# bwa-mem2/bwa-mem2

Hardware: NVIDIA H100
Metric: paired 151bp reads/s (seed+chain+extend hot path) (higher is better)
Workload: dtype int64/int16

## Files before the change

bwa-mem2_b200/csrc/pipeline.cu:

```cuda
#include "bm2_common.cuh"
#include "bm2_ctx.h"
#include "fm_device.cuh"
#include "chain_device.cuh"
#include "ext_device.cuh"
#include <cub/device/device_radix_sort.cuh>
#include <cub/device/device_scan.cuh>
#include <vector>
#include <algorithm>
#include <mutex>
#include <thread>
#include <string>
#include <cstring>
#include <cstdlib>
#include <cmath>

static_assert(sizeof(ExtJobRec) == sizeof(BswJob), "ExtJobRec must alias BswJob");

int bsw_launch_with_scratch(bm2_ctx *ctx_for_error, cudaStream_t stream, const BswJob *d_jobs, BswOut *d_out, int n,
                            const uint8_t *d_tbase, const uint8_t *d_qbase, const BswParams &prm,
                            unsigned long long *d_cells, void *scratch, size_t scratch_bytes, int wide_possible);

__global__ void occ_relayout_kernel(ulonglong2 *tab, size_t n_entries) {
    const size_t i = (size_t) blockIdx.x * blockDim.x + threadIdx.x;
    if (i >= n_entries) return;
// ... 369 lines not shown
    const int r = perm[t];
    const int64_t c0 = chain_off[r], c1 = chain_off[r + 1];
    if (c1 == c0) return;
    const int64_t g0 = reg_off[r];
    ext_build_read_d(cv, ep, chains + c0, (int) (c1 - c0), seeds, (int) (offs[r + 1] - offs[r]), offs[r], c0, g0, b.regs + g0,
                     b.reg_chain + g0, b.reg_seed + g0, b.left + left_off[r], b.left_reg + left_off[r], b.right + right_off[r],
                     b.right_reg + right_off[r], b.srt + g0, b.state ? b.state + g0 : nullptr);
}

__global__ void right_h0_kernel(ExtJobRec *jobs, const int32_t *job_reg, int n, const bm2_alnreg_t *regs) {
    int i = blockIdx.x * blockDim.x + threadIdx.x;
    if (i < n) jobs[i].h0 = regs[job_reg[i]].score;
}

__global__ void fold_kernel(ExtParams ep, const ExtJobRec *jobs, const int32_t *job_reg, const BswOut *outs, const int32_t *sel, int n,
                            int is_right, int w, int last_try, bm2_alnreg_t *regs, const int32_t *reg_chain, const bm2_chain *chains,
                            const bm2_seed *seeds, const int64_t *offs, int32_t *retry, Counters *cnt)
{
    int t = blockIdx.x * blockDim.x + threadIdx.x;
    if (t >= n) return;
    const int j = sel ? sel[t] : t;
    const BswOut o = outs[t];
    const int g = job_reg[j];
    const bm2_chain c = chains[reg_chain[g]];
    const int l_query = (int) (offs[c.seqid + 1] - offs[c.seqid]);
    bm2_alnreg_t a = regs[g];
    const bool ok = ext_fold_d(ep, a, is_right, jobs[j].h0, o.score, o.qle, o.tle, o.gtle, o.gscore, o.max_off, w, last_try, l_query,
                               seeds + c.seed_off, c.n_seeds);
    regs[g] = a;
    if (!ok) { unsigned long long k = atomicAdd(&cnt->n_retry, 1ULL); retry[k] = j; }
}

__global__ void gather_jobs_kernel(const ExtJobRec *jobs, const int32_t *sel, int n, ExtJobRec *out) {
    int t = blockIdx.x * blockDim.x + threadIdx.x;
    if (t < n) out[t] = jobs[sel[t]];
}

__global__ void ext_select_kernel(const ExtJobRec *__restrict__ jobs, const int32_t *__restrict__ job_reg, int n,
                                  const uint8_t *__restrict__ state, int last, ExtJobRec *out, int32_t *out_reg, unsigned long long *n_out)
{
    const int i = blockIdx.x * blockDim.x + threadIdx.x, lane = threadIdx.x & 31;
    int g = 0;
    bool take = false;
    if (i < n) { g = job_reg[i]; const uint8_t s = state[g]; take = s == EXT_NEED || (last && s == EXT_TODO); }
    const unsigned m = __ballot_sync(0xffffffffu, take);
    if (!m) return;
    const int leader = __ffs(m) - 1;
    unsigned long long at = 0;
    if (lane == leader) at = atomicAdd(n_out, (unsigned long long) __popc(m));
    at = __shfl_sync(0xffffffffu, at, leader);
    if (take) { const unsigned long long k = at + __popc(m & ((1u << lane) - 1u)); out[k] = jobs[i]; out_reg[k] = g; }
}

__global__ void ext_mark_done_kernel(uint8_t *state, int64_t n) {
    const int64_t i = (int64_t) blockIdx.x * blockDim.x + threadIdx.x;
    if (i < n && state[i] == EXT_NEED) state[i] = EXT_DONE;
}

__global__ void __launch_bounds__(128)
ext_walk_kernel(ExtParams ep, const bm2_chain *__restrict__ chains, const bm2_seed *__restrict__ seeds, const int64_t *__restrict__ chain_off,
                const int64_t *__restrict__ reg_off, const int64_t *__restrict__ offs, int n_reads, const bm2_alnreg_t *regs,
                const int32_t *__restrict__ reg_seed, uint8_t *state, int32_t *srt2_all, PfBox *box_all, PfCursor *cur, int first, int heavy,
                Counters *cnt)
{
    const int r = blockIdx.x * blockDim.x + threadIdx.x;
    bool done = false;
    if (r < n_reads) {
        const int64_t c0 = chain_off[r], c1 = chain_off[r + 1], g0 = reg_off[r];
        const int n_reg = (int) (reg_off[r + 1] - g0), n_chain = (int) (c1 - c0);
        if (n_chain > 0 && n_reg <= heavy) {
            PfCursor c;
            if (first) { c.ci = 0; c.k = -1; c.lim = 0; c.base = 0; } else c = cur[r];
            if (c.ci < n_chain) {
                done = ext_walk_read_d(ep, chains + c0, n_chain, seeds, (int) (offs[r + 1] - offs[r]), regs + g0, n_reg, reg_seed + g0,
                                       state + g0, srt2_all + g0, box_all + g0, c);
                cur[r] = c;
            }
        }
    }
    if (first) {
        const unsigned m = __ballot_sync(0xffffffffu, done);
        if ((threadIdx.x & 31) == 0 && m) atomicAdd(&cnt->n_walk_done, (unsigned long long) __popc(m));
    }
}

__device__ void ext_postfilter_read_warp(const ExtParams &p, const bm2_chain *chains, int n_chain, const bm2_seed *seeds, int l_query,
                                         bm2_alnreg_t *regs, int n_reg, const int32_t *reg_seed, int32_t *srt2, PfBox *box)
{
    const int lane = threadIdx.x & 31;
    for (int i = lane; i < n_reg; i += 32) box[i] = pf_box_d(regs[i]);
    __syncwarp();
    int lim = 0, base = 0;
    for (int ci = 0; ci < n_chain; ++ci) {
        const bm2_chain &c = chains[ci];
        const bm2_seed *cs = seeds + c.seed_off;
        const int n = c.n_seeds;
        if (n == 0) continue;
        for (int k = n - 1 - lane; k >= 0; k -= 32) srt2[k] = reg_seed[base + (n - 1 - k)];
        __syncwarp();
        for (int k = n - 1; k >= 0; --k) {
            const bm2_seed s = cs[srt2[k]];
            int v = 0;
            bool hit = false;
            for (int i0 = 0; i0 < n_reg && v < lim && !hit; i0 += 128) {
                int kind[4];
#pragma unroll
                for (int g = 0; g < 4; ++g) {
                    const int i = i0 + 32 * g + lane;
                    kind[g] = i < n_reg ? pf_box_kind_d(p, s, box[i], l_query) : 0;
                }
#pragma unroll
                for (int g = 0; g < 4; ++g) {
                    const unsigned cm = __ballot_sync(0xFFFFFFFFu, kind[g] == 1), hm = __ballot_sync(0xFFFFFFFFu, kind[g] == 2);
                    if (hit || v >= lim || i0 + 32 * g >= n_reg) continue;
                    if (hm) {
                        const int at = v + __popc(cm & ((1u << (__ffs(hm) - 1)) - 1u));
                        if (at < lim) { v = at; hit = true; continue; }
                    }
                    v += __popc(cm);
                }
            }
            if (v < lim) {
                if (!pf_chain_overlap_d(cs, n, srt2, k, s)) {
                    __syncwarp();
                    if (lane == 0) {
                        const int ai = base + (n - 1 - k);
                        regs[ai].qb = regs[ai].qe = -1;
                        box[ai].qb = box[ai].qe = -1;
                        srt2[k] = -1;
                    }
                    __syncwarp();
                    continue;
                }
            }
            lim++;
        }
        __syncwarp();
        base += n;
    }
}


__device__ int tail_compact_warp(bm2_alnreg_t *a, int n, int lane) {
    int m = 0;
    for (int i0 = 0; i0 < n; i0 += 32) {
        const int i = i0 + lane;
        uint4 v[7];
        bool keep = false;
        if (i < n) {
            const uint4 *s4 = reinterpret_cast<const uint4 *>(a + i);
#pragma unroll
            for (int k = 0; k < 7; ++k) v[k] = s4[k];
            keep = a[i].qe > a[i].qb;
        }
        const unsigned km = __ballot_sync(0xffffffffu, keep);
        __syncwarp();
        if (keep) {
            const int d = m + __popc(km & ((1u << lane) - 1u));
            if (d != i) {
                uint4 *d4 = reinterpret_cast<uint4 *>(a + d);
#pragma unroll
                for (int k = 0; k < 7; ++k) d4[k] = v[k];
            }
        }
        m += __popc(km);
        __syncwarp();
    }
    return m;
}

__device__ void tail_permute_warp(bm2_alnreg_t *a, int32_t *idx, int n, int lane) {
    for (int i = 0; i < n; ++i) {
        const int first = idx[i];
        if (first < 0 || first == i) continue;
        uint4 tmp = make_uint4(0, 0, 0, 0);
        if (lane < 7) tmp = reinterpret_cast<const uint4 *>(a + i)[lane];
        int j = i;
        for (;;) {
            const int src = idx[j];
            __syncwarp();
            if (lane == 0) idx[j] = -1;
            if (src == i) { if (lane < 7) reinterpret_cast<uint4 *>(a + j)[lane] = tmp; break; }
            if (lane < 7) reinterpret_cast<uint4 *>(a + j)[lane] = reinterpret_cast<const uint4 *>(a + src)[lane];
            j = src;
        }
        __syncwarp();
    }
}

__device__ int ext_tail_read_warp(const ContigView &cv, const ExtParams &p, const uint8_t *ref, const uint8_t *query, bm2_alnreg_t *a, int n_reg,
                                  int32_t *he, int32_t *idx, TailSortKey *keys)
{
    const int lane = threadIdx.x & 31;
    int n = tail_compact_warp(a, n_reg, lane);
    if (n > 1) {
        for (int i = lane; i < n; i += 32) { idx[i] = i; keys[i].r = a[i].re; }
        __syncwarp();
        if (lane == 0) {
            const TailSortKey *rk = keys;
            ks_introsort_d(idx, (long) n, [rk](int x, int y) { return rk[x].r < rk[y].r; });
        }
        __syncwarp();
        tail_permute_warp(a, idx, n, lane);
        for (int i = lane; i < n; i += 32) reg_set_n_comp_d(a[i], 1);
        __syncwarp();
        if (lane == 0) sort_dedup_scan_d(cv, p, ref, query, n, a, he);
        __syncwarp();
        n = tail_compact_warp(a, n, lane);
        for (int i = lane; i < n; i += 32) { idx[i] = i; keys[i].r = a[i].rb; keys[i].score = a[i].score; keys[i].qb = a[i].qb; }
        __syncwarp();
        if (lane == 0) {
            const TailSortKey *rk = keys;
            ks_introsort_d(idx, (long) n, [rk](int xi, int yi) {
                const TailSortKey x = rk[xi], y = rk[yi];
                return x.score > y.score || (x.score == y.score && (x.r < y.r || (x.r == y.r && x.qb < y.qb)));
            });
        }
        __syncwarp();
        tail_permute_warp(a, idx, n, lane);
        for (int i0 = 0; i0 < n; i0 += 32) {
            const int i = i0 + lane;
            const bool dup = i >= 1 && i < n && a[i].score == a[i - 1].score && a[i].rb == a[i - 1].rb && a[i].qb == a[i - 1].qb;
            __syncwarp();
            if (dup) a[i].qe = a[i].qb;
        }
        __syncwarp();
        if (n > 1) n = 1 + tail_compact_warp(a + 1, n - 1, lane);
    }
    for (int i = lane; i < n; i += 32)
        if (a[i].rid >= 0 && cv.ann_alt && cv.ann_alt[a[i].rid]) reg_set_is_alt_d(a[i], 1);
    __syncwarp();
    return n;
}

template <int mode>
__global__ void __launch_bounds__(128, mode ? 4 : 1)
tail_kernel(ContigView cv, ExtParams ep, const uint8_t *__restrict__ ref, const uint8_t *__restrict__ codes, const int64_t *__restrict__ offs,
            const bm2_chain *__restrict__ chains, const bm2_seed *__restrict__ seeds, const int64_t *__restrict__ chain_off,
            const int64_t *__restrict__ reg_off, int n_reads, bm2_alnreg_t *regs, const int32_t *reg_seed, int32_t *srt2_all, int32_t *he_all,
            int he_stride, const int32_t *__restrict__ perm, PfBox *box_all, int32_t *n_final, int heavy_thr, int light_sorted, int coop_tail)
{
    const int tid = blockIdx.x * blockDim.x + threadIdx.x, nthr = gridDim.x * blockDim.x;
    const int lane = threadIdx.x & 31;
    int32_t *he = he_all + (size_t) (mode ? tid >> 5 : tid) * he_stride;
    const int unit = mode ? tid >> 5 : tid, nunit = mode ? nthr >> 5 : nthr;
    for (int t = unit; t < n_reads; t += nunit) {
        const int r = (mode || light_sorted) ? perm[t] : t;
        const int64_t c0 = chain_off[r], c1 = chain_off[r + 1], g0 = reg_off[r];
        const int n_reg = (int) (reg_off[r + 1] - g0);
        if (mode) { if (n_reg <= heavy_thr) break; }
        else if (n_reg > heavy_thr) continue;
        int m = 0;
        if (c1 > c0) {
            const int l_query = (int) (offs[r + 1] - offs[r]);
            if (mode) {
                ext_postfilter_read_warp(ep, chains + c0, (int) (c1 - c0), seeds, l_query, regs + g0, n_reg, reg_seed + g0, srt2_all + g0, box_all + g0);
                __syncwarp();
                if (coop_tail) m = ext_tail_read_warp(cv, ep, ref, codes + offs[r], regs + g0, n_reg, he, srt2_all + g0, reinterpret_cast<TailSortKey *>(box_all + g0));
                else if (lane == 0) m = ext_tail_read_d(cv, ep, ref, codes + offs[r], regs + g0, n_reg, he, srt2_all + g0, reinterpret_cast<TailSortKey *>(box_all + g0));
                __syncwarp();
            } else {
                ext_postfilter_read_d(ep, chains + c0, (int) (c1 - c0), seeds, l_query, regs + g0, n_reg, reg_seed + g0, srt2_all + g0, box_all + g0);
                m = ext_tail_read_d(cv, ep, ref, codes + offs[r], regs + g0, n_reg, he, srt2_all + g0, reinterpret_cast<TailSortKey *>(box_all + g0));
            }
        }
        if (!mode || lane == 0) n_final[r] = m;
    }
}

__global__ void regs_gather_kernel(const bm2_alnreg_t *regs, const int64_t *reg_off, const int64_t *out_off, int n_reads, bm2_alnreg_t *out) {
    const int r = blockIdx.x * blockDim.x + threadIdx.x;
    if (r >= n_reads) return;
    const int64_t o0 = out_off[r], o1 = out_off[r + 1], g0 = reg_off[r];
    for (int64_t k = 0; k < o1 - o0; ++k) reg_copy(&out[o0 + k], &regs[g0 + k]);
}

__global__ void work_keys_slots_kernel(const int64_t *read_smem_off, const int64_t *slot_off, int n, uint32_t *keys, int32_t *vals) {
    int r = blockIdx.x * blockDim.x + threadIdx.x;
    if (r >= n) return;
    int64_t w = slot_off[read_smem_off[r + 1]] - slot_off[read_smem_off[r]];
    keys[r] = 0xFFFFFFFFu - (uint32_t) (w > 0x7FFFFFFF ? 0x7FFFFFFF : w);
    vals[r] = r;
}
__global__ void work_keys_off_kernel(const int64_t *off, int n, uint32_t *keys, int32_t *vals) {
    int r = blockIdx.x * blockDim.x + threadIdx.x;
    if (r >= n) return;
    int64_t w = off[r + 1] - off[r];
    keys[r] = 0xFFFFFFFFu - (uint32_t) (w > 0x7FFFFFFF ? 0x7FFFFFFF : w);
    vals[r] = r;
}

__global__ void widen_kernel(const int32_t *in, int n, int64_t *out) {
    int i = blockIdx.x * blockDim.x + threadIdx.x;
    if (i < n) out[i] = in[i];
    if (i == n) out[i] = 0;
}

namespace {
enum Buf {
    B_CODES, B_OFFS, B_CNT, B_PREV, B_RESEED, B_SMEM_RAW, B_KEYS_IN, B_KEYS_OUT, B_VALS_IN, B_VALS_OUT, B_CUB, B_SMEM, B_SLOT_CNT,
    B_SLOT_OFF, B_READ_SMEM_OFF, B_SA, B_WSEED, B_WCHAIN, B_ORD, B_SRT, B_KV, B_FIN_CHAIN, B_FIN_SEED, B_PER_READ, B_SCAN, B_CHAINS,
    B_SEEDS, B_REGS, B_REG_AUX, B_JOBS, B_NW, B_OUT, B_PERM, B_ORDPOS, B_FLT, B_MINHSP, B_OWNER, B_POOL, B_TASKS, B_RTASKS, B_COUNT_
};
static_assert(B_COUNT_ <= 64, "bm2_ctx::d[] too small");
enum HBuf { H_OUT_REGS, H_OUT_OFF, H_SMEM, H_CHAINS, H_SEEDS, H_MISC };

struct Stages {
    bm2_ctx *ctx; std::vector<cudaEvent_t> &ev; std::vector<const char *> &names;
    int n = 0;
    int mark(const char *name) {
        bm2_ctx *ctx_for_error = ctx;
        if ((int) ev.size() <= n) { cudaEvent_t e; BM2_CUDA_OK(cudaEventCreate(&e)); ev.push_back(e); }
        BM2_CUDA_OK(cudaEventRecord(ev[n], ctx->stream));
        if ((int) names.size() <= n) names.push_back(name); else names[n] = name;
        ++n;
// ... 241 lines not shown
    char *prb = (char *) ctx->d[B_PER_READ].p;
    int32_t *d_nchain = (int32_t *) prb, *d_nseed = (int32_t *) (prb + pr), *d_nleft = (int32_t *) (prb + 2 * pr),
            *d_nright = (int32_t *) (prb + 3 * pr), *d_nfinal = (int32_t *) (prb + 4 * pr);
    ChainBufs cb = { P<WSeed>(ctx, B_WSEED), P<WChain>(ctx, B_WCHAIN), P<int32_t>(ctx, B_ORD), P<int32_t>(ctx, B_SRT), P<int32_t>(ctx, B_KV),
                     P<int64_t>(ctx, B_ORDPOS), P<FltRec>(ctx, B_FLT),
                     P<bm2_chain>(ctx, B_FIN_CHAIN), P<bm2_seed>(ctx, B_FIN_SEED), d_nchain, d_nseed, d_nleft, d_nright };
    if (ctx->ensure(ctx->d[B_PERM], al((size_t) n * 4) * 4)) return 1;
    uint32_t *wk_in = (uint32_t *) ctx->d[B_PERM].p, *wk_out = (uint32_t *) ((char *) ctx->d[B_PERM].p + al((size_t) n * 4));
    int32_t *wv_in = (int32_t *) ((char *) ctx->d[B_PERM].p + 2 * al((size_t) n * 4)), *d_perm = (int32_t *) ((char *) ctx->d[B_PERM].p + 3 * al((size_t) n * 4));
    work_keys_slots_kernel<<<(n + 255) / 256, 256, 0, st>>>(P<int64_t>(ctx, B_READ_SMEM_OFF), P<int64_t>(ctx, B_SLOT_OFF), n, wk_in, wv_in);
    if (sort_work(ctx, wk_in, wk_out, wv_in, d_perm, n, true)) return 1;
    const int light_sorted = env_int("BM2_LIGHT_SORTED", 0, 0, 1);
    const int chain_heavy = env_int("BM2_CHAIN_HEAVY", 64, 1, 1 << 30);
    const int chain_coop_min = env_int("BM2_CHAIN_COOP_MIN", 1024, 0, 1 << 30);
    chain_kernel<<<(n + 127) / 128, 128, 0, st>>>(pv.cv, pv.cp, P<bm2_smem>(ctx, B_SMEM), P<int64_t>(ctx, B_READ_SMEM_OFF),
                                                  P<int64_t>(ctx, B_SLOT_OFF), P<int64_t>(ctx, B_SA), d_offs, n, d_perm, cb, pv.sw, ctx->idx.ref, d_codes,
                                                  any_flt ? P<int32_t>(ctx, B_MINHSP) : nullptr, 0, chain_heavy, chain_coop_min, light_sorted);
    {
        int heavy_warps = n < ctx->n_sm * 256 ? n : ctx->n_sm * 256;
        chain_kernel<<<(heavy_warps * 32 + 127) / 128, 128, 0, st>>>(pv.cv, pv.cp, P<bm2_smem>(ctx, B_SMEM), P<int64_t>(ctx, B_READ_SMEM_OFF),
                                                                      P<int64_t>(ctx, B_SLOT_OFF), P<int64_t>(ctx, B_SA), d_offs, n, d_perm, cb, pv.sw,
                                                                      ctx->idx.ref, d_codes, any_flt ? P<int32_t>(ctx, B_MINHSP) : nullptr, 1, chain_heavy, chain_coop_min, 0);
    }

    if (sg.mark("compact")) return 1;
    const size_t sc = al((size_t) (n + 2) * 8);
    char *scb = (char *) ctx->d[B_SCAN].p;
    int64_t *w_tmp = (int64_t *) scb, *d_chain_off = (int64_t *) (scb + sc), *d_reg_off = (int64_t *) (scb + 2 * sc),
            *d_left_off = (int64_t *) (scb + 3 * sc), *d_right_off = (int64_t *) (scb + 4 * sc), *d_out_off = (int64_t *) (scb + 5 * sc);
    const int gw = (n + 1 + 255) / 256;
    widen_kernel<<<gw, 256, 0, st>>>(d_nchain, n, w_tmp); if (scan64(ctx, w_tmp, d_chain_off, n)) return 1;
    widen_kernel<<<gw, 256, 0, st>>>(d_nseed, n, w_tmp);  if (scan64(ctx, w_tmp, d_reg_off, n)) return 1;
    widen_kernel<<<gw, 256, 0, st>>>(d_nleft, n, w_tmp);  if (scan64(ctx, w_tmp, d_left_off, n)) return 1;
    widen_kernel<<<gw, 256, 0, st>>>(d_nright, n, w_tmp); if (scan64(ctx, w_tmp, d_right_off, n)) return 1;
    int64_t tot[4];
    BM2_CUDA_OK(cudaMemcpyAsync(&tot[0], d_chain_off + n, 8, cudaMemcpyDeviceToHost, st));
    BM2_CUDA_OK(cudaMemcpyAsync(&tot[1], d_reg_off + n, 8, cudaMemcpyDeviceToHost, st));
    BM2_CUDA_OK(cudaMemcpyAsync(&tot[2], d_left_off + n, 8, cudaMemcpyDeviceToHost, st));
    BM2_CUDA_OK(cudaMemcpyAsync(&tot[3], d_right_off + n, 8, cudaMemcpyDeviceToHost, st));
    BM2_CUDA_OK(cudaMemcpyAsync(&h_cnt, d_cnt, sizeof(Counters), cudaMemcpyDeviceToHost, st));
    BM2_CUDA_OK(cudaStreamSynchronize(st));
    ctx->last_n_lf = h_cnt.n_lf;
    const int64_t n_chains = tot[0], n_regs = tot[1], n_left = tot[2], n_right = tot[3];
    bs.n_chains = n_chains; bs.n_regs = n_regs; bs.n_left = n_left; bs.n_right = n_right;
    if (n_regs > 2000000000LL) { bm2_set_error(ctx, "too many seeds in one batch"); return 1; }
    if (ctx->ensure(ctx->d[B_CHAINS], (size_t) (n_chains + 1) * sizeof(bm2_chain)) || ctx->ensure(ctx->d[B_SEEDS], (size_t) (n_regs + 1) * sizeof(bm2_seed))) return 1;
    chain_compact_kernel<<<(n + 127) / 128, 128, 0, st>>>(P<int64_t>(ctx, B_READ_SMEM_OFF), P<int64_t>(ctx, B_SLOT_OFF), n, P<bm2_chain>(ctx, B_FIN_CHAIN),
                                                          P<bm2_seed>(ctx, B_FIN_SEED), d_chain_off, d_reg_off, P<bm2_chain>(ctx, B_CHAINS), P<bm2_seed>(ctx, B_SEEDS));
    if (upto == UPTO_CHAIN) { if (sg.mark("end")) return 1; BM2_CUDA_OK(cudaStreamSynchronize(st)); return 0; }

    if (sg.mark("extbuild")) return 1;
    const size_t nr1 = (size_t) n_regs + 1, nl1 = (size_t) n_left + 1, nrt1 = (size_t) n_right + 1;
    const int lazy = env_int("BM2_EXT_LAZY", 1, 0, 1);
    const int waves = env_int("BM2_EXT_WAVES", 2, 2, 64);
    const size_t aux_bytes = al(nr1 * 4) * 3 + al(nr1 * 8) + al(nl1 * 4) * 2 + al(nrt1 * 4) * 2 + al(nr1 * sizeof(PfBox)) +
                             (lazy ? al(nr1) + al((size_t) n * sizeof(PfCursor)) + al(nl1 * 4) + al(nrt1 * 4) : 0);
    const size_t njmax = nl1 > nrt1 ? nl1 : nrt1;
    if (ctx->ensure(ctx->d[B_REGS], nr1 * sizeof(bm2_alnreg_t)) || ctx->ensure(ctx->d[B_REG_AUX], aux_bytes) ||
        ctx->ensure(ctx->d[B_JOBS], al(nl1 * sizeof(ExtJobRec)) + al(nrt1 * sizeof(ExtJobRec)) + al(njmax * sizeof(ExtJobRec)) + al(njmax * sizeof(BswOut)) +
                                    (lazy ? al(nl1 * sizeof(ExtJobRec)) + al(nrt1 * sizeof(ExtJobRec)) : 0)) ||
        ctx->ensure(ctx->bsw_scratch, bsw_scratch_bytes((int) njmax))) return 1;
    char *ab = (char *) ctx->d[B_REG_AUX].p;
    int32_t *d_reg_chain = (int32_t *) ab; ab += al(nr1 * 4);
    int32_t *d_reg_seed = (int32_t *) ab; ab += al(nr1 * 4);
    int32_t *d_srt2 = (int32_t *) ab; ab += al(nr1 * 4);
    uint64_t *d_srt = (uint64_t *) ab; ab += al(nr1 * 8);
    int32_t *d_left_reg = (int32_t *) ab; ab += al(nl1 * 4);
    int32_t *d_left_retry = (int32_t *) ab; ab += al(nl1 * 4);
    int32_t *d_right_reg = (int32_t *) ab; ab += al(nrt1 * 4);
    int32_t *d_right_retry = (int32_t *) ab; ab += al(nrt1 * 4);
    PfBox *d_box = (PfBox *) ab; ab += al(nr1 * sizeof(PfBox));
    uint8_t *d_state = nullptr; PfCursor *d_cursor = nullptr; int32_t *d_wleft_reg = nullptr, *d_wright_reg = nullptr;
    if (lazy) {
        d_state = (uint8_t *) ab; ab += al(nr1);
        d_cursor = (PfCursor *) ab; ab += al((size_t) n * sizeof(PfCursor));
        d_wleft_reg = (int32_t *) ab; ab += al(nl1 * 4);
        d_wright_reg = (int32_t *) ab; ab += al(nrt1 * 4);
    }
    char *jb = (char *) ctx->d[B_JOBS].p;
    ExtJobRec *d_left = (ExtJobRec *) jb; jb += al(nl1 * sizeof(ExtJobRec));
    ExtJobRec *d_right = (ExtJobRec *) jb; jb += al(nrt1 * sizeof(ExtJobRec));
    ExtJobRec *d_retry_jobs = (ExtJobRec *) jb; jb += al(njmax * sizeof(ExtJobRec));
    BswOut *d_outs = (BswOut *) jb; jb += al(njmax * sizeof(BswOut));
    ExtJobRec *d_wleft = nullptr, *d_wright = nullptr;
    if (lazy) { d_wleft = (ExtJobRec *) jb; jb += al(nl1 * sizeof(ExtJobRec)); d_wright = (ExtJobRec *) jb; }
    bm2_alnreg_t *d_regs = P<bm2_alnreg_t>(ctx, B_REGS);
    ExtBufs eb = { d_regs, d_reg_chain, d_reg_seed, d_srt, d_left, d_right, d_left_reg, d_right_reg, d_state };
    work_keys_off_kernel<<<(n + 255) / 256, 256, 0, st>>>(d_reg_off, n, wk_in, wv_in);
    if (sort_work(ctx, wk_in, wk_out, wv_in, d_perm, n)) return 1;
    ext_build_kernel<<<(n + 127) / 128, 128, 0, st>>>(pv.cv, pv.ep, P<bm2_chain>(ctx, B_CHAINS), P<bm2_seed>(ctx, B_SEEDS), d_chain_off, d_reg_off,
                                                      d_left_off, d_right_off, d_offs, n, d_perm, eb);

    auto phase = [&](const char *name, ExtJobRec *jobs, int32_t *job_reg, int32_t *retry, int64_t nj, int is_right) -> int {
        if (sg.mark(name)) return 1;
        if (nj <= 0) return 0;
        StageToken tok_bsw((use_tokens & 2) ? &ctx->parent->tok_bsw : nullptr);
        BswParams bp; bp.a = ctx->opt.a; bp.b = ctx->opt.b; bp.o_del = ctx->opt.o_del; bp.e_del = ctx->opt.e_del; bp.o_ins = ctx->opt.o_ins;
        bp.e_ins = ctx->opt.e_ins; bp.zdrop = ctx->opt.zdrop; bp.end_bonus = is_right ? ctx->opt.pen_clip3 : ctx->opt.pen_clip5; bp.w = ctx->opt.w;
        if (is_right) right_h0_kernel<<<(unsigned) ((nj + 255) / 256), 256, 0, st>>>(jobs, job_reg, (int) nj, d_regs);
        BM2_CUDA_OK(cudaMemsetAsync(&d_cnt->n_retry, 0, 8, st));
        if (bsw_launch_with_scratch(ctx, st, (const BswJob *) jobs, d_outs, (int) nj, ctx->idx.ref, d_codes, bp, &d_cnt->cells, ctx->bsw_scratch.p,
                                    ctx->bsw_scratch.cap, 1)) return 1;
        fold_kernel<<<(unsigned) ((nj + 255) / 256), 256, 0, st>>>(pv.ep, jobs, job_reg, d_outs, nullptr, (int) nj, is_right, bp.w, 0, d_regs, d_reg_chain,
                                                                   P<bm2_chain>(ctx, B_CHAINS), P<bm2_seed>(ctx, B_SEEDS), d_offs, retry, d_cnt);
        unsigned long long n_retry = 0;
        BM2_CUDA_OK(cudaMemcpyAsync(&n_retry, &d_cnt->n_retry, 8, cudaMemcpyDeviceToHost, st));
        BM2_CUDA_OK(cudaStreamSynchronize(st));
        if (n_retry > 0) {
            gather_jobs_kernel<<<(unsigned) ((n_retry + 255) / 256), 256, 0, st>>>(jobs, retry, (int) n_retry, d_retry_jobs);
            bp.w = ctx->opt.w << 1;
            if (bsw_launch_with_scratch(ctx, st, (const BswJob *) d_retry_jobs, d_outs, (int) n_retry, ctx->idx.ref, d_codes, bp, &d_cnt->cells,
                                        ctx->bsw_scratch.p, ctx->bsw_scratch.cap, 1)) return 1;
            fold_kernel<<<(unsigned) ((n_retry + 255) / 256), 256, 0, st>>>(pv.ep, jobs, job_reg, d_outs, retry, (int) n_retry, is_right, bp.w, 1, d_regs,
                                                                            d_reg_chain, P<bm2_chain>(ctx, B_CHAINS), P<bm2_seed>(ctx, B_SEEDS), d_offs,
                                                                            retry, d_cnt);
        }
        ctx->last_n_retry[is_right] += n_retry;
        return 0;
    };
    ctx->last_n_retry[0] = ctx->last_n_retry[1] = 0;
    ctx->last_jobs_skipped = 0;
    if (!lazy) {
        if (phase("bsw_left", d_left, d_left_reg, d_left_retry, n_left, 0)) return 1;
        if (phase("bsw_right", d_right, d_right_reg, d_right_retry, n_right, 1)) return 1;
    } else {
        int64_t jobs_run = 0;
        const int walk_heavy = env_int("BM2_EXT_WALK_HEAVY", 256, 0, 1 << 30);
        for (int wave = 1; wave <= waves; ++wave) {
            const int last = wave == waves;
            if (sg.mark("ext_select")) return 1;
            BM2_CUDA_OK(cudaMemsetAsync(d_cnt->n_sel, 0, sizeof(d_cnt->n_sel), st));
            if (n_left > 0)
                ext_select_kernel<<<(unsigned) ((n_left + 255) / 256), 256, 0, st>>>(d_left, d_left_reg, (int) n_left, d_state, last, d_wleft,
                                                                                     d_wleft_reg, &d_cnt->n_sel[0]);
            if (n_right > 0)
                ext_select_kernel<<<(unsigned) ((n_right + 255) / 256), 256, 0, st>>>(d_right, d_right_reg, (int) n_right, d_state, last, d_wright,
                                                                                      d_wright_reg, &d_cnt->n_sel[1]);
            unsigned long long n_sel[2] = {0, 0};
            BM2_CUDA_OK(cudaMemcpyAsync(n_sel, d_cnt->n_sel, sizeof(n_sel), cudaMemcpyDeviceToHost, st));
            BM2_CUDA_OK(cudaStreamSynchronize(st));
            if (phase("bsw_left", d_wleft, d_wleft_reg, d_left_retry, (int64_t) n_sel[0], 0)) return 1;
            if (phase("bsw_right", d_wright, d_wright_reg, d_right_retry, (int64_t) n_sel[1], 1)) return 1;
            jobs_run += (int64_t) (n_sel[0] + n_sel[1]);
            if (last) break;
            if (sg.mark("ext_walk")) return 1;
            ext_mark_done_kernel<<<(unsigned) ((n_regs + 255) / 256), 256, 0, st>>>(d_state, n_regs);
            ext_walk_kernel<<<(n + 127) / 128, 128, 0, st>>>(pv.ep, P<bm2_chain>(ctx, B_CHAINS), P<bm2_seed>(ctx, B_SEEDS), d_chain_off, d_reg_off, d_offs, n,
                                                             d_regs, d_reg_seed, d_state, d_srt2, d_box, d_cursor, wave == 1, walk_heavy, d_cnt);
        }
        ctx->last_jobs_skipped = (unsigned long long) (n_left + n_right - jobs_run);
    }

    if (sg.mark("tail")) return 1;
    int blocks_i = (n + 127) / 128; const int max_blocks_i = ctx->n_sm * 8; if (blocks_i > max_blocks_i) blocks_i = max_blocks_i;
    const int he_stride = 2 * (max_len + 2);
    if (ctx->ensure(ctx->d[B_NW], (size_t) blocks_i * 128 * he_stride * 4)) return 1;
    const int heavy_thr = env_int("BM2_TAIL_HEAVY", 24, 1, 1 << 20);
    work_keys_off_kernel<<<(n + 255) / 256, 256, 0, st>>>(d_reg_off, n, wk_in, wv_in);
    if (sort_work(ctx, wk_in, wk_out, wv_in, d_perm, n, true)) return 1;
    if (getenv("BM2_DEBUG_NREG")) {
        std::vector<int64_t> ho((size_t) n + 1);
        BM2_CUDA_OK(cudaMemcpyAsync(ho.data(), d_reg_off, (size_t) (n + 1) * 8, cudaMemcpyDeviceToHost, st));
        BM2_CUDA_OK(cudaStreamSynchronize(st));
        std::vector<int64_t> cntv((size_t) n);
        for (int i = 0; i < n; ++i) cntv[i] = ho[i + 1] - ho[i];
        std::sort(cntv.begin(), cntv.end(), [](int64_t a, int64_t b) { return a > b; });
        long long c24 = 0, c256 = 0, c1024 = 0; double sq = 0;
        for (int i = 0; i < n; ++i) { c24 += cntv[i] > 24; c256 += cntv[i] > 256; c1024 += cntv[i] > 1024; if (cntv[i] > 24) sq += (double) cntv[i] * (double) cntv[i]; }
        fprintf(stderr, "[bm2 debug] regs before the tail: reads %d, > 24: %lld, > 256: %lld, > 1024: %lld, sum of squares over the heavy reads %.3g; heaviest:", n, c24, c256, c1024, sq);
        for (int i = 0; i < 8 && i < n; ++i) fprintf(stderr, " %lld", (long long) cntv[i]);
        fprintf(stderr, "\n");
    }
    tail_kernel<0><<<blocks_i, 128, 0, st>>>(pv.cv, pv.ep, ctx->idx.ref, d_codes, d_offs, P<bm2_chain>(ctx, B_CHAINS), P<bm2_seed>(ctx, B_SEEDS), d_chain_off,
                                             d_reg_off, n, d_regs, d_reg_seed, d_srt2, P<int32_t>(ctx, B_NW), he_stride, d_perm, d_box, d_nfinal, heavy_thr, light_sorted, 0);
    tail_kernel<1><<<blocks_i, 128, 0, st>>>(pv.cv, pv.ep, ctx->idx.ref, d_codes, d_offs, P<bm2_chain>(ctx, B_CHAINS), P<bm2_seed>(ctx, B_SEEDS), d_chain_off,
                                             d_reg_off, n, d_regs, d_reg_seed, d_srt2, P<int32_t>(ctx, B_NW), he_stride, d_perm, d_box, d_nfinal, heavy_thr, 0, env_int("BM2_TAIL_COOP", 1, 0, 1));

    if (sg.mark("output")) return 1;
    widen_kernel<<<gw, 256, 0, st>>>(d_nfinal, n, w_tmp); if (scan64(ctx, w_tmp, d_out_off, n)) return 1;
    if (ctx->ensure(ctx->d[B_OUT], nr1 * sizeof(bm2_alnreg_t))) return 1;
    regs_gather_kernel<<<(n + 127) / 128, 128, 0, st>>>(d_regs, d_reg_off, d_out_off, n, P<bm2_alnreg_t>(ctx, B_OUT));
    if (ctx->ensure_host(ctx->h[H_OUT_OFF], (size_t) (n + 1) * 8)) return 1;
    BM2_CUDA_OK(cudaMemcpyAsync(ctx->h[H_OUT_OFF].p, d_out_off, (size_t) (n + 1) * 8, cudaMemcpyDeviceToHost, st));
    BM2_CUDA_OK(cudaMemcpyAsync(&h_cnt, d_cnt, sizeof(Counters), cudaMemcpyDeviceToHost, st));
    BM2_CUDA_OK(cudaStreamSynchronize(st));
    ctx->last_cells = h_cnt.cells;
    ctx->last_walk_done = h_cnt.n_walk_done;
    const int64_t n_out = ((const int64_t *) ctx->h[H_OUT_OFF].p)[n];
    bs.n_out = n_out;
    if (copy_out && ctx->ensure_host(ctx->h[H_OUT_REGS], (size_t) (n_out + 1) * sizeof(bm2_alnreg_t))) return 1;
    if (n_out && copy_out) BM2_CUDA_OK(cudaMemcpyAsync(ctx->h[H_OUT_REGS].p, ctx->d[B_OUT].p, (size_t) n_out * sizeof(bm2_alnreg_t), cudaMemcpyDeviceToHost, st));
    if (sg.mark("end")) return 1;
    BM2_CUDA_OK(cudaStreamSynchronize(st));
    BM2_CUDA_OK(cudaGetLastError());
    return 0;
}

int finish_stage_times(bm2_ctx *ctx) {
    bm2_ctx *ctx_for_error = ctx;
    ctx->stage_ms.clear();
    size_t n = ctx->stage_names.size();
    size_t marks = 0;
    for (; marks < n; ++marks) if (strcmp(ctx->stage_names[marks], "end") == 0) { ++marks; break; }
    std::vector<const char *> names;
    for (size_t i = 0; i < marks; ++i) {
        float ms = 0;
        if (i + 1 < marks) BM2_CUDA_OK(cudaEventElapsedTime(&ms, ctx->events[i], ctx->events[i + 1]));
        size_t j = 0;
        while (j < names.size() && strcmp(names[j], ctx->stage_names[i]) != 0) ++j;
        if (j == names.size()) { names.push_back(ctx->stage_names[i]); ctx->stage_ms.push_back(0.f); }
        ctx->stage_ms[j] += ms;
    }
    ctx->stage_names = names;
    return 0;
}

}

extern "C" int bm2_collect_smems(bm2_ctx *ctx, const bm2_read_batch *reads, bm2_smem_result *out) {
    bm2_ctx *ctx_for_error = ctx;
    if (!ctx || !reads || !out) return 1;
    BatchState bs;
    if (run_pipeline(ctx, reads, UPTO_SMEM, bs)) return 1;
    finish_stage_times(ctx);
    if (ctx->ensure_host(ctx->h[H_SMEM], (size_t) (bs.n_smem + 1) * sizeof(bm2_smem)) || ctx->ensure_host(ctx->h[H_OUT_OFF], (size_t) (bs.n + 2) * 8)) return 1;
    if (bs.n_smem) BM2_CUDA_OK(cudaMemcpy(ctx->h[H_SMEM].p, ctx->d[B_SMEM].p, (size_t) bs.n_smem * sizeof(bm2_smem), cudaMemcpyDeviceToHost));
    if (bs.n > 0) BM2_CUDA_OK(cudaMemcpy(ctx->h[H_OUT_OFF].p, ctx->d[B_READ_SMEM_OFF].p, (size_t) (bs.n + 1) * 8, cudaMemcpyDeviceToHost));
    else ((int64_t *) ctx->h[H_OUT_OFF].p)[0] = 0;
    out->n = bs.n_smem; out->smems = (const bm2_smem *) ctx->h[H_SMEM].p; out->read_off = (const int64_t *) ctx->h[H_OUT_OFF].p;
// ... 145 lines not shown
```

Before: 9.716 million.

## Fold post-filter into lazy extension walk and add warp-cooperative walk for heavy reads

Removes the separate post-filter pass from the tail kernels. The lazy extension walk now decides purging for every read: a per-thread kernel handles light reads and a new warp-per-read kernel handles heavy reads via the sorted permutation. The walk runs after every wave, including the last one, and the tail only applies the recorded purge marks from the box array. Heavy reads were previously excluded from lazy skipping (walk_heavy 256), so they can now skip more extension jobs. The cost is an extra walk launch per wave, an earlier sort and memset, and lazy buffers that are always allocated.

```diff
diff --git a/bwa-mem2_b200/csrc/pipeline.cu b/bwa-mem2_b200/csrc/pipeline.cu
--- a/bwa-mem2_b200/csrc/pipeline.cu
+++ b/bwa-mem2_b200/csrc/pipeline.cu
@@ -445,91 +445,126 @@
     if (take) { const unsigned long long k = at + __popc(m & ((1u << lane) - 1u)); out[k] = jobs[i]; out_reg[k] = g; }
 }
 
-__global__ void ext_mark_done_kernel(uint8_t *state, int64_t n) {
+__global__ void ext_mark_done_kernel(uint8_t *state, int64_t n, int last) {
     const int64_t i = (int64_t) blockIdx.x * blockDim.x + threadIdx.x;
-    if (i < n && state[i] == EXT_NEED) state[i] = EXT_DONE;
-}
-
-__global__ void __launch_bounds__(128)
-ext_walk_kernel(ExtParams ep, const bm2_chain *__restrict__ chains, const bm2_seed *__restrict__ seeds, const int64_t *__restrict__ chain_off,
-                const int64_t *__restrict__ reg_off, const int64_t *__restrict__ offs, int n_reads, const bm2_alnreg_t *regs,
-                const int32_t *__restrict__ reg_seed, uint8_t *state, int32_t *srt2_all, PfBox *box_all, PfCursor *cur, int first, int heavy,
-                Counters *cnt)
-{
-    const int r = blockIdx.x * blockDim.x + threadIdx.x;
-    bool done = false;
-    if (r < n_reads) {
-        const int64_t c0 = chain_off[r], c1 = chain_off[r + 1], g0 = reg_off[r];
-        const int n_reg = (int) (reg_off[r + 1] - g0), n_chain = (int) (c1 - c0);
-        if (n_chain > 0 && n_reg <= heavy) {
-            PfCursor c;
-            if (first) { c.ci = 0; c.k = -1; c.lim = 0; c.base = 0; } else c = cur[r];
-            if (c.ci < n_chain) {
-                done = ext_walk_read_d(ep, chains + c0, n_chain, seeds, (int) (offs[r + 1] - offs[r]), regs + g0, n_reg, reg_seed + g0,
-                                       state + g0, srt2_all + g0, box_all + g0, c);
-                cur[r] = c;
+    if (i < n && (state[i] == EXT_NEED || (last && state[i] == EXT_TODO))) state[i] = EXT_DONE;
+}
+
+__device__ bool pf_seed_purged_warp(const ExtParams &p, const bm2_seed *cs, int n, const int32_t *srt2, int k, int l_query, const PfBox *box,
+                                    int n_reg, int lim)
+{
+    const int lane = threadIdx.x & 31;
+    const bm2_seed s = cs[srt2[k]];
+    int v = 0;
+    bool hit = false;
+    for (int i0 = 0; i0 < n_reg && v < lim && !hit; i0 += 128) {
+        int kind[4];
+#pragma unroll
+        for (int g = 0; g < 4; ++g) {
+            const int i = i0 + 32 * g + lane;
+            kind[g] = i < n_reg ? pf_box_kind_d(p, s, box[i], l_query) : 0;
+        }
+#pragma unroll
+        for (int g = 0; g < 4; ++g) {
+            const unsigned cm = __ballot_sync(0xFFFFFFFFu, kind[g] == 1), hm = __ballot_sync(0xFFFFFFFFu, kind[g] == 2);
+            if (hit || v >= lim || i0 + 32 * g >= n_reg) continue;
+            if (hm) {
+                const int at = v + __popc(cm & ((1u << (__ffs(hm) - 1)) - 1u));
+                if (at < lim) { v = at; hit = true; continue; }
             }
-        }
-    }
-    if (first) {
-        const unsigned m = __ballot_sync(0xffffffffu, done);
-        if ((threadIdx.x & 31) == 0 && m) atomicAdd(&cnt->n_walk_done, (unsigned long long) __popc(m));
-    }
-}
-
-__device__ void ext_postfilter_read_warp(const ExtParams &p, const bm2_chain *chains, int n_chain, const bm2_seed *seeds, int l_query,
-                                         bm2_alnreg_t *regs, int n_reg, const int32_t *reg_seed, int32_t *srt2, PfBox *box)
+            v += __popc(cm);
+        }
+    }
+    return v < lim && !pf_chain_overlap_d(cs, n, srt2, k, s);
+}
+
+__device__ bool ext_walk_read_warp(const ExtParams &p, const bm2_chain *chains, int n_chain, const bm2_seed *seeds, int l_query,
+                                   const bm2_alnreg_t *regs, int n_reg, const int32_t *reg_seed, uint8_t *state, int32_t *srt2, PfBox *box,
+                                   PfCursor &cur)
 {
     const int lane = threadIdx.x & 31;
-    for (int i = lane; i < n_reg; i += 32) box[i] = pf_box_d(regs[i]);
-    __syncwarp();
-    int lim = 0, base = 0;
-    for (int ci = 0; ci < n_chain; ++ci) {
+    int ci = cur.ci, k = cur.k, lim = cur.lim, base = cur.base;
+    for (; ci < n_chain; ++ci, k = -1) {
         const bm2_chain &c = chains[ci];
         const bm2_seed *cs = seeds + c.seed_off;
         const int n = c.n_seeds;
         if (n == 0) continue;
-        for (int k = n - 1 - lane; k >= 0; k -= 32) srt2[k] = reg_seed[base + (n - 1 - k)];
-        __syncwarp();
-        for (int k = n - 1; k >= 0; --k) {
-            const bm2_seed s = cs[srt2[k]];
-            int v = 0;
-            bool hit = false;
-            for (int i0 = 0; i0 < n_reg && v < lim && !hit; i0 += 128) {
-                int kind[4];
-#pragma unroll
-                for (int g = 0; g < 4; ++g) {
-                    const int i = i0 + 32 * g + lane;
-                    kind[g] = i < n_reg ? pf_box_kind_d(p, s, box[i], l_query) : 0;
+        if (k < 0) {
+            for (int kk = n - 1 - lane; kk >= 0; kk -= 32) srt2[kk] = reg_seed[base + (n - 1 - kk)];
+            __syncwarp();
+            k = n - 1;
+        }
+        for (; k >= 0; --k) {
+            const int ai = base + (n - 1 - k);
+            const bool extended = state[ai] == EXT_DONE;
+            const bool purged = pf_seed_purged_warp(p, cs, n, srt2, k, l_query, box, n_reg, lim);
+            __syncwarp();
+            if (purged) {
+                if (lane == 0) {
+                    box[ai].qb = box[ai].qe = -1;
+                    srt2[k] = -1;
+                    if (!extended) state[ai] = EXT_SKIP;
                 }
-#pragma unroll
-                for (int g = 0; g < 4; ++g) {
-                    const unsigned cm = __ballot_sync(0xFFFFFFFFu, kind[g] == 1), hm = __ballot_sync(0xFFFFFFFFu, kind[g] == 2);
-                    if (hit || v >= lim || i0 + 32 * g >= n_reg) continue;
-                    if (hm) {
-                        const int at = v + __popc(cm & ((1u << (__ffs(hm) - 1)) - 1u));
-                        if (at < lim) { v = at; hit = true; continue; }
-                    }
-                    v += __popc(cm);
+                __syncwarp();
+                continue;
+            }
+            if (!extended) {
+                if (lane == 0) state[ai] = EXT_NEED;
+                cur.ci = ci; cur.k = k; cur.lim = lim; cur.base = base;
+                return false;
+            }
+            if (lane == 0) box[ai] = pf_box_d(regs[ai]);
+            __syncwarp();
+            lim++;
+        }
+        base += n;
+    }
+    cur.ci = ci; cur.k = -1; cur.lim = lim; cur.base = base;
+    return true;
+}
+
+template <int mode>
+__global__ void __launch_bounds__(128)
+ext_walk_kernel(ExtParams ep, const bm2_chain *__restrict__ chains, const bm2_seed *__restrict__ seeds, const int64_t *__restrict__ chain_off,
+                const int64_t *__restrict__ reg_off, const int64_t *__restrict__ offs, int n_reads, const int32_t *__restrict__ perm,
+                const bm2_alnreg_t *regs, const int32_t *__restrict__ reg_seed, uint8_t *state, int32_t *srt2_all, PfBox *box_all, PfCursor *cur,
+                int first, int heavy_thr, Counters *cnt)
+{
+    const int tid = blockIdx.x * blockDim.x + threadIdx.x, lane = threadIdx.x & 31;
+    unsigned n_done = 0;
+    if (!mode) {
+        const int r = tid;
+        if (r < n_reads) {
+            const int64_t c0 = chain_off[r], c1 = chain_off[r + 1], g0 = reg_off[r];
+            const int n_reg = (int) (reg_off[r + 1] - g0), n_chain = (int) (c1 - c0);
+            if (n_chain > 0 && n_reg <= heavy_thr) {
+                PfCursor c;
+                if (first) { c.ci = 0; c.k = -1; c.lim = 0; c.base = 0; } else c = cur[r];
+                if (c.ci < n_chain) {
+                    n_done = ext_walk_read_d(ep, chains + c0, n_chain, seeds, (int) (offs[r + 1] - offs[r]), regs + g0, n_reg, reg_seed + g0,
+                                             state + g0, srt2_all + g0, box_all + g0, c);
+                    cur[r] = c;
                 }
             }
-            if (v < lim) {
-                if (!pf_chain_overlap_d(cs, n, srt2, k, s)) {
-                    __syncwarp();
-                    if (lane == 0) {
-                        const int ai = base + (n - 1 - k);
-                        regs[ai].qb = regs[ai].qe = -1;
-                        box[ai].qb = box[ai].qe = -1;
-                        srt2[k] = -1;
-                    }
-                    __syncwarp();
-                    continue;
-                }
+        }
+    } else {
+        for (int t = tid >> 5; t < n_reads; t += (gridDim.x * blockDim.x) >> 5) {
+            const int r = perm[t];
+            const int64_t c0 = chain_off[r], c1 = chain_off[r + 1], g0 = reg_off[r];
+            const int n_reg = (int) (reg_off[r + 1] - g0), n_chain = (int) (c1 - c0);
+            if (n_reg <= heavy_thr) break;
+            PfCursor c;
+            if (first) { c.ci = 0; c.k = -1; c.lim = 0; c.base = 0; } else c = cur[r];
+            if (c.ci < n_chain) {
+                const bool done = ext_walk_read_warp(ep, chains + c0, n_chain, seeds, (int) (offs[r + 1] - offs[r]), regs + g0, n_reg,
+                                                     reg_seed + g0, state + g0, srt2_all + g0, box_all + g0, c);
+                if (lane == 0) { cur[r] = c; n_done += done; }
             }
-            lim++;
-        }
-        __syncwarp();
-        base += n;
+        }
+    }
+    if (cnt) {
+        n_done = __reduce_add_sync(0xffffffffu, n_done);
+        if (lane == 0 && n_done) atomicAdd(&cnt->n_walk_done, (unsigned long long) n_done);
     }
 }
 
@@ -629,9 +664,9 @@
 template <int mode>
 __global__ void __launch_bounds__(128, mode ? 4 : 1)
 tail_kernel(ContigView cv, ExtParams ep, const uint8_t *__restrict__ ref, const uint8_t *__restrict__ codes, const int64_t *__restrict__ offs,
-            const bm2_chain *__restrict__ chains, const bm2_seed *__restrict__ seeds, const int64_t *__restrict__ chain_off,
-            const int64_t *__restrict__ reg_off, int n_reads, bm2_alnreg_t *regs, const int32_t *reg_seed, int32_t *srt2_all, int32_t *he_all,
-            int he_stride, const int32_t *__restrict__ perm, PfBox *box_all, int32_t *n_final, int heavy_thr, int light_sorted, int coop_tail)
+            const int64_t *__restrict__ chain_off, const int64_t *__restrict__ reg_off, int n_reads, bm2_alnreg_t *regs, int32_t *srt2_all,
+            int32_t *he_all, int he_stride, const int32_t *__restrict__ perm, PfBox *box_all, int32_t *n_final, int heavy_thr, int light_sorted,
+            int coop_tail)
 {
     const int tid = blockIdx.x * blockDim.x + threadIdx.x, nthr = gridDim.x * blockDim.x;
     const int lane = threadIdx.x & 31;
@@ -645,15 +680,16 @@
         else if (n_reg > heavy_thr) continue;
         int m = 0;
         if (c1 > c0) {
-            const int l_query = (int) (offs[r + 1] - offs[r]);
+            bm2_alnreg_t *a = regs + g0;
+            const PfBox *box = box_all + g0;
             if (mode) {
-                ext_postfilter_read_warp(ep, chains + c0, (int) (c1 - c0), seeds, l_query, regs + g0, n_reg, reg_seed + g0, srt2_all + g0, box_all + g0);
+                for (int i = lane; i < n_reg; i += 32) if (box[i].qb == -1 && box[i].qe == -1) a[i].qb = a[i].qe = -1;
                 __syncwarp();
                 if (coop_tail) m = ext_tail_read_warp(cv, ep, ref, codes + offs[r], regs + g0, n_reg, he, srt2_all + g0, reinterpret_cast<TailSortKey *>(box_all + g0));
                 else if (lane == 0) m = ext_tail_read_d(cv, ep, ref, codes + offs[r], regs + g0, n_reg, he, srt2_all + g0, reinterpret_cast<TailSortKey *>(box_all + g0));
                 __syncwarp();
             } else {
-                ext_postfilter_read_d(ep, chains + c0, (int) (c1 - c0), seeds, l_query, regs + g0, n_reg, reg_seed + g0, srt2_all + g0, box_all + g0);
+                for (int i = 0; i < n_reg; ++i) if (box[i].qb == -1 && box[i].qe == -1) a[i].qb = a[i].qe = -1;
                 m = ext_tail_read_d(cv, ep, ref, codes + offs[r], regs + g0, n_reg, he, srt2_all + g0, reinterpret_cast<TailSortKey *>(box_all + g0));
             }
         }
@@ -1001,13 +1037,13 @@
     if (sg.mark("extbuild")) return 1;
     const size_t nr1 = (size_t) n_regs + 1, nl1 = (size_t) n_left + 1, nrt1 = (size_t) n_right + 1;
     const int lazy = env_int("BM2_EXT_LAZY", 1, 0, 1);
-    const int waves = env_int("BM2_EXT_WAVES", 2, 2, 64);
+    const int waves = lazy ? env_int("BM2_EXT_WAVES", 2, 2, 64) : 1;
     const size_t aux_bytes = al(nr1 * 4) * 3 + al(nr1 * 8) + al(nl1 * 4) * 2 + al(nrt1 * 4) * 2 + al(nr1 * sizeof(PfBox)) +
-                             (lazy ? al(nr1) + al((size_t) n * sizeof(PfCursor)) + al(nl1 * 4) + al(nrt1 * 4) : 0);
+                             al(nr1) + al((size_t) n * sizeof(PfCursor)) + al(nl1 * 4) + al(nrt1 * 4);
     const size_t njmax = nl1 > nrt1 ? nl1 : nrt1;
     if (ctx->ensure(ctx->d[B_REGS], nr1 * sizeof(bm2_alnreg_t)) || ctx->ensure(ctx->d[B_REG_AUX], aux_bytes) ||
-        ctx->ensure(ctx->d[B_JOBS], al(nl1 * sizeof(ExtJobRec)) + al(nrt1 * sizeof(ExtJobRec)) + al(njmax * sizeof(ExtJobRec)) + al(njmax * sizeof(BswOut)) +
-                                    (lazy ? al(nl1 * sizeof(ExtJobRec)) + al(nrt1 * sizeof(ExtJobRec)) : 0)) ||
+        ctx->ensure(ctx->d[B_JOBS], al(nl1 * sizeof(ExtJobRec)) * 2 + al(nrt1 * sizeof(ExtJobRec)) * 2 + al(njmax * sizeof(ExtJobRec)) +
+                                    al(njmax * sizeof(BswOut))) ||
         ctx->ensure(ctx->bsw_scratch, bsw_scratch_bytes((int) njmax))) return 1;
     char *ab = (char *) ctx->d[B_REG_AUX].p;
     int32_t *d_reg_chain = (int32_t *) ab; ab += al(nr1 * 4);
@@ -1019,26 +1055,27 @@
     int32_t *d_right_reg = (int32_t *) ab; ab += al(nrt1 * 4);
     int32_t *d_right_retry = (int32_t *) ab; ab += al(nrt1 * 4);
     PfBox *d_box = (PfBox *) ab; ab += al(nr1 * sizeof(PfBox));
-    uint8_t *d_state = nullptr; PfCursor *d_cursor = nullptr; int32_t *d_wleft_reg = nullptr, *d_wright_reg = nullptr;
-    if (lazy) {
-        d_state = (uint8_t *) ab; ab += al(nr1);
-        d_cursor = (PfCursor *) ab; ab += al((size_t) n * sizeof(PfCursor));
-        d_wleft_reg = (int32_t *) ab; ab += al(nl1 * 4);
-        d_wright_reg = (int32_t *) ab; ab += al(nrt1 * 4);
-    }
+    uint8_t *d_state = (uint8_t *) ab; ab += al(nr1);
+    PfCursor *d_cursor = (PfCursor *) ab; ab += al((size_t) n * sizeof(PfCursor));
+    int32_t *d_wleft_reg = (int32_t *) ab; ab += al(nl1 * 4);
+    int32_t *d_wright_reg = (int32_t *) ab; ab += al(nrt1 * 4);
     char *jb = (char *) ctx->d[B_JOBS].p;
     ExtJobRec *d_left = (ExtJobRec *) jb; jb += al(nl1 * sizeof(ExtJobRec));
     ExtJobRec *d_right = (ExtJobRec *) jb; jb += al(nrt1 * sizeof(ExtJobRec));
     ExtJobRec *d_retry_jobs = (ExtJobRec *) jb; jb += al(njmax * sizeof(ExtJobRec));
     BswOut *d_outs = (BswOut *) jb; jb += al(njmax * sizeof(BswOut));
-    ExtJobRec *d_wleft = nullptr, *d_wright = nullptr;
-    if (lazy) { d_wleft = (ExtJobRec *) jb; jb += al(nl1 * sizeof(ExtJobRec)); d_wright = (ExtJobRec *) jb; }
+    ExtJobRec *d_wleft = (ExtJobRec *) jb; jb += al(nl1 * sizeof(ExtJobRec));
+    ExtJobRec *d_wright = (ExtJobRec *) jb;
     bm2_alnreg_t *d_regs = P<bm2_alnreg_t>(ctx, B_REGS);
     ExtBufs eb = { d_regs, d_reg_chain, d_reg_seed, d_srt, d_left, d_right, d_left_reg, d_right_reg, d_state };
     work_keys_off_kernel<<<(n + 255) / 256, 256, 0, st>>>(d_reg_off, n, wk_in, wv_in);
     if (sort_work(ctx, wk_in, wk_out, wv_in, d_perm, n)) return 1;
     ext_build_kernel<<<(n + 127) / 128, 128, 0, st>>>(pv.cv, pv.ep, P<bm2_chain>(ctx, B_CHAINS), P<bm2_seed>(ctx, B_SEEDS), d_chain_off, d_reg_off,
                                                       d_left_off, d_right_off, d_offs, n, d_perm, eb);
+    if (sort_work(ctx, wk_in, wk_out, wv_in, d_perm, n, true)) return 1;
+    BM2_CUDA_OK(cudaMemsetAsync(d_box, 0xFF, nr1 * sizeof(PfBox), st));
+    const int heavy_thr = env_int("BM2_TAIL_HEAVY", 24, 1, 1 << 20);
+    int blocks_i = (n + 127) / 128; const int max_blocks_i = ctx->n_sm * 8; if (blocks_i > max_blocks_i) blocks_i = max_blocks_i;
 
     auto phase = [&](const char *name, ExtJobRec *jobs, int32_t *job_reg, int32_t *retry, int64_t nj, int is_right) -> int {
         if (sg.mark(name)) return 1;
@@ -1068,45 +1105,38 @@
         return 0;
     };
     ctx->last_n_retry[0] = ctx->last_n_retry[1] = 0;
-    ctx->last_jobs_skipped = 0;
-    if (!lazy) {
-        if (phase("bsw_left", d_left, d_left_reg, d_left_retry, n_left, 0)) return 1;
-        if (phase("bsw_right", d_right, d_right_reg, d_right_retry, n_right, 1)) return 1;
-    } else {
-        int64_t jobs_run = 0;
-        const int walk_heavy = env_int("BM2_EXT_WALK_HEAVY", 256, 0, 1 << 30);
-        for (int wave = 1; wave <= waves; ++wave) {
-            const int last = wave == waves;
-            if (sg.mark("ext_select")) return 1;
-            BM2_CUDA_OK(cudaMemsetAsync(d_cnt->n_sel, 0, sizeof(d_cnt->n_sel), st));
-            if (n_left > 0)
-                ext_select_kernel<<<(unsigned) ((n_left + 255) / 256), 256, 0, st>>>(d_left, d_left_reg, (int) n_left, d_state, last, d_wleft,
-                                                                                     d_wleft_reg, &d_cnt->n_sel[0]);
-            if (n_right > 0)
-                ext_select_kernel<<<(unsigned) ((n_right + 255) / 256), 256, 0, st>>>(d_right, d_right_reg, (int) n_right, d_state, last, d_wright,
-                                                                                      d_wright_reg, &d_cnt->n_sel[1]);
-            unsigned long long n_sel[2] = {0, 0};
-            BM2_CUDA_OK(cudaMemcpyAsync(n_sel, d_cnt->n_sel, sizeof(n_sel), cudaMemcpyDeviceToHost, st));
-            BM2_CUDA_OK(cudaStreamSynchronize(st));
-            if (phase("bsw_left", d_wleft, d_wleft_reg, d_left_retry, (int64_t) n_sel[0], 0)) return 1;
-            if (phase("bsw_right", d_wright, d_wright_reg, d_right_retry, (int64_t) n_sel[1], 1)) return 1;
-            jobs_run += (int64_t) (n_sel[0] + n_sel[1]);
-            if (last) break;
-            if (sg.mark("ext_walk")) return 1;
-            ext_mark_done_kernel<<<(unsigned) ((n_regs + 255) / 256), 256, 0, st>>>(d_state, n_regs);
-            ext_walk_kernel<<<(n + 127) / 128, 128, 0, st>>>(pv.ep, P<bm2_chain>(ctx, B_CHAINS), P<bm2_seed>(ctx, B_SEEDS), d_chain_off, d_reg_off, d_offs, n,
-                                                             d_regs, d_reg_seed, d_state, d_srt2, d_box, d_cursor, wave == 1, walk_heavy, d_cnt);
-        }
-        ctx->last_jobs_skipped = (unsigned long long) (n_left + n_right - jobs_run);
-    }
+    auto walk = [&](int first, Counters *count) {
+        ext_walk_kernel<0><<<(n + 127) / 128, 128, 0, st>>>(pv.ep, P<bm2_chain>(ctx, B_CHAINS), P<bm2_seed>(ctx, B_SEEDS), d_chain_off, d_reg_off, d_offs,
+                                                            n, d_perm, d_regs, d_reg_seed, d_state, d_srt2, d_box, d_cursor, first, heavy_thr, count);
+        ext_walk_kernel<1><<<blocks_i, 128, 0, st>>>(pv.ep, P<bm2_chain>(ctx, B_CHAINS), P<bm2_seed>(ctx, B_SEEDS), d_chain_off, d_reg_off, d_offs,
+                                                     n, d_perm, d_regs, d_reg_seed, d_state, d_srt2, d_box, d_cursor, first, heavy_thr, count);
+    };
+    int64_t jobs_run = 0;
+    for (int wave = 1; wave <= waves; ++wave) {
+        const int last = wave == waves;
+        if (sg.mark("ext_select")) return 1;
+        BM2_CUDA_OK(cudaMemsetAsync(d_cnt->n_sel, 0, sizeof(d_cnt->n_sel), st));
+        if (n_left > 0)
+            ext_select_kernel<<<(unsigned) ((n_left + 255) / 256), 256, 0, st>>>(d_left, d_left_reg, (int) n_left, d_state, last, d_wleft,
+                                                                                 d_wleft_reg, &d_cnt->n_sel[0]);
+        if (n_right > 0)
+            ext_select_kernel<<<(unsigned) ((n_right + 255) / 256), 256, 0, st>>>(d_right, d_right_reg, (int) n_right, d_state, last, d_wright,
+                                                                                  d_wright_reg, &d_cnt->n_sel[1]);
+        unsigned long long n_sel[2] = {0, 0};
+        BM2_CUDA_OK(cudaMemcpyAsync(n_sel, d_cnt->n_sel, sizeof(n_sel), cudaMemcpyDeviceToHost, st));
+        BM2_CUDA_OK(cudaStreamSynchronize(st));
+        if (phase("bsw_left", d_wleft, d_wleft_reg, d_left_retry, (int64_t) n_sel[0], 0)) return 1;
+        if (phase("bsw_right", d_wright, d_wright_reg, d_right_retry, (int64_t) n_sel[1], 1)) return 1;
+        jobs_run += (int64_t) (n_sel[0] + n_sel[1]);
+        if (sg.mark("ext_walk")) return 1;
+        if (n_regs > 0) ext_mark_done_kernel<<<(unsigned) ((n_regs + 255) / 256), 256, 0, st>>>(d_state, n_regs, last);
+        walk(wave == 1, (wave == 1 && !last) ? d_cnt : nullptr);
+    }
+    ctx->last_jobs_skipped = (unsigned long long) (n_left + n_right - jobs_run);
 
     if (sg.mark("tail")) return 1;
-    int blocks_i = (n + 127) / 128; const int max_blocks_i = ctx->n_sm * 8; if (blocks_i > max_blocks_i) blocks_i = max_blocks_i;
     const int he_stride = 2 * (max_len + 2);
     if (ctx->ensure(ctx->d[B_NW], (size_t) blocks_i * 128 * he_stride * 4)) return 1;
-    const int heavy_thr = env_int("BM2_TAIL_HEAVY", 24, 1, 1 << 20);
-    work_keys_off_kernel<<<(n + 255) / 256, 256, 0, st>>>(d_reg_off, n, wk_in, wv_in);
-    if (sort_work(ctx, wk_in, wk_out, wv_in, d_perm, n, true)) return 1;
     if (getenv("BM2_DEBUG_NREG")) {
         std::vector<int64_t> ho((size_t) n + 1);
         BM2_CUDA_OK(cudaMemcpyAsync(ho.data(), d_reg_off, (size_t) (n + 1) * 8, cudaMemcpyDeviceToHost, st));
@@ -1120,10 +1150,10 @@
         for (int i = 0; i < 8 && i < n; ++i) fprintf(stderr, " %lld", (long long) cntv[i]);
         fprintf(stderr, "\n");
     }
-    tail_kernel<0><<<blocks_i, 128, 0, st>>>(pv.cv, pv.ep, ctx->idx.ref, d_codes, d_offs, P<bm2_chain>(ctx, B_CHAINS), P<bm2_seed>(ctx, B_SEEDS), d_chain_off,
-                                             d_reg_off, n, d_regs, d_reg_seed, d_srt2, P<int32_t>(ctx, B_NW), he_stride, d_perm, d_box, d_nfinal, heavy_thr, light_sorted, 0);
-    tail_kernel<1><<<blocks_i, 128, 0, st>>>(pv.cv, pv.ep, ctx->idx.ref, d_codes, d_offs, P<bm2_chain>(ctx, B_CHAINS), P<bm2_seed>(ctx, B_SEEDS), d_chain_off,
-                                             d_reg_off, n, d_regs, d_reg_seed, d_srt2, P<int32_t>(ctx, B_NW), he_stride, d_perm, d_box, d_nfinal, heavy_thr, 0, env_int("BM2_TAIL_COOP", 1, 0, 1));
+    tail_kernel<0><<<blocks_i, 128, 0, st>>>(pv.cv, pv.ep, ctx->idx.ref, d_codes, d_offs, d_chain_off, d_reg_off, n, d_regs, d_srt2,
+                                             P<int32_t>(ctx, B_NW), he_stride, d_perm, d_box, d_nfinal, heavy_thr, light_sorted, 0);
+    tail_kernel<1><<<blocks_i, 128, 0, st>>>(pv.cv, pv.ep, ctx->idx.ref, d_codes, d_offs, d_chain_off, d_reg_off, n, d_regs, d_srt2,
+                                             P<int32_t>(ctx, B_NW), he_stride, d_perm, d_box, d_nfinal, heavy_thr, 0, env_int("BM2_TAIL_COOP", 1, 0, 1));
 
     if (sg.mark("output")) return 1;
     widen_kernel<<<gw, 256, 0, st>>>(d_nfinal, n, w_tmp); if (scan64(ctx, w_tmp, d_out_off, n)) return 1;
```

After: 10.89 million, median of 6. +12.1%, better.
